# ETM-Code/eirgrid

Measured on AMD Instinct MI355X. Metric: 26-year episodes/sec, higher is better.
Workload: dtype f64

## Files before the change

eirgrid_amd/_native.py:

```python
from __future__ import annotations

import ctypes as C
import os

YEARS, N_ACTIONS, N_DEFICIT, N_COUNTS, N_TYPES = 26, 61, 15, 21, 15
GRID, CELLS, YEARLY_FIELDS = 51, 2601, 21
MAX_GENS, MAX_OFFSETS, RUN_CAP, DEF_CAP, ACT_CAP, ONCHIP_GENS = 4096, 4096, 4096, 4096, 4096, 512
TOPK_MAX = 64
PARETO_MAX = 256
PARETO_KEEP_SPREAD = 0x100
STATS_LEN = 8 + 2 * YEARS * N_ACTIONS + YEARS * N_DEFICIT
CANDIDATE_BYTES = 8 + 8 + 32 + 4 * YEARS + 4 * YEARS + RUN_CAP + DEF_CAP
PACKET_BYTES = 8 * STATS_LEN + CANDIDATE_BYTES

EG_OK, EG_ERR_NO_DEVICE, EG_ERR_BAD_ARG, EG_ERR_HIP, EG_ERR_UNSUPPORTED, EG_ERR_NOMEM, EG_ERR_INTERNAL = 0, -1, -2, -3, -4, -5, -6
EG_EP_OK, EG_EP_OVERFLOW, EG_EP_NO_LOCATION, EG_EP_INTERNAL = 0, -1, -2, -3

LIB_PATH = os.environ.get("EIRGRID_LIB") or os.path.join(os.path.dirname(os.path.abspath(__file__)), "libeirgrid_hip.so")

_dp = C.POINTER(C.c_double)
_u8p = C.POINTER(C.c_uint8)
_u16p = C.POINTER(C.c_uint16)
_u32p = C.POINTER(C.c_uint32)
_i32p = C.POINTER(C.c_int32)
# ... 123 lines not shown
DEBUG_TURNOVER_BREED, DEBUG_TURNOVER_EXPLORE = 1, 2
DEBUG_PARETO_ENTRY_BYTES = 56
DEBUG_PARETO_STATE_BYTES = 32 + PARETO_MAX * DEBUG_PARETO_ENTRY_BYTES
DEBUG_BREED_HEADER_BYTES, DEBUG_BREED_ROW_BYTES = 32, 288
DEBUG_BREED_READBACK_BYTES = DEBUG_BREED_HEADER_BYTES + PARETO_MAX * DEBUG_BREED_ROW_BYTES
DEBUG_BREED_BLOCK_OFFSETS = 416


class EgUpdateCandidate(C.Structure):
    _fields_ = [("score", C.c_double), ("index", C.c_int64), ("metrics", C.c_double * 4), ("n_run", C.c_int32 * YEARS), ("n_def", C.c_int32 * YEARS),
                ("run_log", C.c_uint8 * RUN_CAP), ("def_log", C.c_uint8 * DEF_CAP)]


class EgDebugRefineEntry(C.Structure):
    _fields_ = [("winner", C.c_int32), ("n_failed", C.c_int32), ("edit", C.c_uint32 * 2), ("score", C.c_double), ("metrics", C.c_double * 4),
                ("off26", C.c_int32), ("offd26", C.c_int32), ("base_ok", C.c_int32), ("n", C.c_int32), ("base_score", C.c_double),
                ("base_metrics", C.c_double * 4)]


assert C.sizeof(EgUpdateCandidate) == CANDIDATE_BYTES and C.sizeof(EgDebugRefineEntry) == 112

EXPORTS = [
    "eg_build_hash", "eg_last_error", "eg_device_count", "eg_create", "eg_destroy", "eg_rollout_batch", "eg_upload_snapshot",
    "eg_rollout_launch", "eg_rollout_launch_update", "eg_sync", "eg_last_batch_size", "eg_policy_hold", "eg_policy_rewind", "eg_replay_hoist", "eg_replay_hoist_stats", "eg_debug_hoist_stamps", "eg_fetch", "eg_timing_reset", "eg_timing_read", "eg_timing_read_grids", "eg_memory_report", "eg_update_stats", "eg_fetch_scores",
    "eg_fetch_episode_lists", "eg_fetch_record", "eg_fetch_best_run", "eg_best_result_track", "eg_fetch_best_result", "eg_evaluate_action_impact", "eg_place", "eg_find_suitable_location", "eg_debug_fill_lds", "eg_debug_occupy", "eg_policy_apply_reduced", "eg_policy_apply_packet", "eg_train_step",
    "eg_policy_push", "eg_device_rollout", "eg_device_apply", "eg_device_step", "eg_policy_pull",
    "eg_group_create", "eg_group_destroy", "eg_group_rank", "eg_group_push", "eg_group_step", "eg_group_pull", "eg_group_replay_hoist",
    "eg_group_best_result_track", "eg_group_fetch_best_result", "eg_top_k_track", "eg_fetch_top_k", "eg_rank_score",
    "eg_pareto_track", "eg_pareto_fold_last_batch", "eg_fetch_pareto", "eg_debug_pareto_fold",
    "eg_debug_load_batch", "eg_debug_fold_last_batch", "eg_debug_pick_best", "eg_debug_refine_pick",
    "eg_group_top_k_track", "eg_group_fetch_top_k", "eg_plans_validate", "eg_evaluate_plans", "eg_plans_load", "eg_plans_free",
    "eg_plan_edits_validate", "eg_evaluate_plan_edits", "eg_debug_fetch_plan_block", "eg_plans_save", "eg_refine_validate", "eg_refine_plan",
    "eg_refine_plans_validate", "eg_refine_plans", "eg_debug_refine_pick_many",
    "eg_debug_breed_begin", "eg_debug_breed_chunk", "eg_debug_breed_turnover", "eg_debug_breed_fetch",
    "eg_plan_moves_validate", "eg_evaluate_plan_moves", "eg_refine_plans_moves_validate", "eg_refine_plans_moves",
    "eg_plan_crosses_validate", "eg_evaluate_plan_crosses", "eg_plan_rewrites_validate", "eg_evaluate_plan_rewrites",
    "eg_breed_validate", "eg_breed_plans", "eg_explore_validate", "eg_explore_neighbourhood", "eg_explore_plans",
    "eg_host_tables_create", "eg_host_tables_free", "eg_host_tables_f64", "eg_host_tables_i32",
    "eg_policy_new", "eg_policy_free", "eg_policy_snapshot_view", "eg_policy_get_tables", "eg_policy_set_tables",
    "eg_policy_get_scalar", "eg_policy_set_scalar", "eg_policy_get_list", "eg_policy_apply_episode", "eg_score_metrics",
    "eg_policy_save_json", "eg_policy_load_json", "eg_policy_append_weight_history", "eg_policy_export_improvement_csv", "eg_export_summary_csv", "eg_export_run_details",
]

_lib = None


def source_hash() -> str:
    import glob
    import hashlib
    csrc = os.path.join(os.path.dirname(os.path.abspath(__file__)), "csrc")
    rel = [os.path.basename(f) for pat in ("*.hip", "*.cpp", "*.h") for f in glob.glob(os.path.join(csrc, pat))]
    rel += ["../../include/" + os.path.basename(f) for f in glob.glob(os.path.join(csrc, "..", "..", "include", "*.h"))]
    rel = sorted(set(rel + ["Makefile"]) - {"eg_build_hash.cpp"}, key=lambda r: r.encode())
    h = hashlib.sha256()
    for r in rel:
        h.update(open(os.path.join(csrc, r), "rb").read())
    return h.hexdigest()[:16]


def lib():
    global _lib
    if _lib is not None:
        return _lib
    if not os.path.exists(LIB_PATH):
        raise ImportError(f"{LIB_PATH} is missing: run `python -c 'import __graft_entry__ as g; g.build()'` "
                          "(hipcc --offload-arch=gfx950).  eirgrid_amd has no CPU fallback.")
    L = C.CDLL(LIB_PATH)
# ... 169 lines not shown
        L.eg_explore_neighbourhood.restype = C.c_int32
        L.eg_explore_neighbourhood.argtypes = [C.POINTER(EgPlanSet), C.POINTER(EgExploreOpts), C.POINTER(C.c_int64)]
        L.eg_explore_plans.restype = C.c_int32
        L.eg_explore_plans.argtypes = [C.c_void_p, C.POINTER(EgPolicySnapshot), C.POINTER(EgOpts), C.POINTER(EgPlanSet), C.POINTER(EgExploreOpts),
                                       C.c_uint64, C.c_uint64, C.POINTER(C.POINTER(EgPlanSet)), C.POINTER(EgExploreGeneration),
                                       C.POINTER(EgExploreMember), C.POINTER(C.c_int64), _i32p, _i32p, C.POINTER(EgEpisodeOut)]
    if hasattr(L, "eg_pareto_track") or not os.environ.get("EIRGRID_LIB"):
        L.eg_pareto_track.restype = C.c_int32
        L.eg_pareto_track.argtypes = [C.c_void_p, C.c_int32, C.c_int32, C.c_int32]
        L.eg_pareto_fold_last_batch.restype = C.c_int32
        L.eg_pareto_fold_last_batch.argtypes = [C.c_void_p]
        L.eg_fetch_pareto.restype = C.c_int32
        L.eg_fetch_pareto.argtypes = [C.c_void_p, C.POINTER(EgEpisodeOut), _i32p, C.POINTER(C.c_int64), _dp, C.POINTER(C.c_int64)]
        L.eg_debug_pareto_fold.restype = C.c_int32
        L.eg_debug_pareto_fold.argtypes = [C.c_void_p, _dp, _i32p, C.c_uint32, C.c_uint64]
    if hasattr(L, "eg_debug_load_batch") or not os.environ.get("EIRGRID_LIB"):
        L.eg_debug_load_batch.restype = C.c_int32
        L.eg_debug_load_batch.argtypes = [C.c_void_p, _dp, _i32p, _i32p, _u8p, _dp, C.c_uint32, C.c_uint64]
        L.eg_debug_fold_last_batch.restype = C.c_int32
        L.eg_debug_fold_last_batch.argtypes = [C.c_void_p, C.c_int32, C.c_int32]
        L.eg_debug_pick_best.restype = C.c_int32
        L.eg_debug_pick_best.argtypes = [C.c_void_p, C.c_void_p]
        L.eg_debug_refine_pick.restype = C.c_int32
        L.eg_debug_refine_pick.argtypes = [C.c_void_p, C.c_int32, C.c_void_p, _u8p]
    if hasattr(L, "eg_debug_breed_begin") or not os.environ.get("EIRGRID_LIB"):
        L.eg_debug_breed_begin.restype = C.c_int32
        L.eg_debug_breed_begin.argtypes = [C.c_void_p, C.c_int32, C.c_int32, C.c_int32]
        L.eg_debug_breed_chunk.restype = C.c_int32
        L.eg_debug_breed_chunk.argtypes = [C.c_void_p, _dp, _i32p, C.c_uint32, C.c_uint64]
        L.eg_debug_breed_turnover.restype = C.c_int32
        L.eg_debug_breed_turnover.argtypes = [C.c_void_p, C.c_int32, C.c_int32, C.c_int64]
        L.eg_debug_breed_fetch.restype = C.c_int32
        L.eg_debug_breed_fetch.argtypes = [C.c_void_p, C.c_void_p, _u8p, _u8p, _u8p, _u8p, C.c_void_p, _u64p]
    L.eg_plans_load.restype = C.POINTER(EgPlanSet)
    L.eg_plans_load.argtypes = [C.c_char_p]
    L.eg_plans_free.argtypes = [C.POINTER(EgPlanSet)]
    L.eg_rank_score.restype = C.c_double
    L.eg_rank_score.argtypes = [_dp, C.c_int32]
    L.eg_evaluate_action_impact.restype = C.c_double
    L.eg_evaluate_action_impact.argtypes = [_dp, _dp, C.c_int32]
    L.eg_fetch_best_run.restype = C.c_int32
    L.eg_fetch_best_run.argtypes = [C.c_void_p, C.POINTER(EgEpisodeOut), C.POINTER(C.c_int32)]
    L.eg_policy_export_improvement_csv.argtypes = [C.c_void_p, C.c_char_p]
    L.eg_find_suitable_location.restype = C.c_int32
    L.eg_find_suitable_location.argtypes = [C.c_void_p, C.c_int32, C.c_int32, _dp, _dp, C.c_int32, C.c_float, _dp, _dp, _i32p, _dp]
    L.eg_place.restype = C.c_int32
    L.eg_debug_fill_lds.restype = C.c_int32
    L.eg_debug_fill_lds.argtypes = [C.c_void_p, C.c_uint32]
    if hasattr(L, "eg_debug_occupy") or not os.environ.get("EIRGRID_LIB"):
        L.eg_debug_occupy.restype = C.c_int32
        L.eg_debug_occupy.argtypes = [C.c_void_p, C.c_int32, C.c_uint64]
    L.eg_place.argtypes = [C.c_void_p, C.c_int32, C.c_int32, _u16p, C.c_int32, _i32p, _dp]
    L.eg_host_tables_create.restype = C.c_void_p
    L.eg_host_tables_create.argtypes = [C.POINTER(EgWorld)]
    L.eg_host_tables_free.argtypes = [C.c_void_p]
    L.eg_host_tables_f64.restype = C.c_int32
    L.eg_host_tables_f64.argtypes = [C.c_void_p, C.c_char_p, C.POINTER(_dp), C.POINTER(C.c_int64)]
    L.eg_host_tables_i32.restype = C.c_int32
    L.eg_host_tables_i32.argtypes = [C.c_void_p, C.c_char_p, C.POINTER(_i32p), C.POINTER(C.c_int64)]
    L.eg_policy_new.restype = C.c_void_p
    L.eg_policy_free.argtypes = [C.c_void_p]
    L.eg_policy_snapshot_view.restype = C.c_int32
    L.eg_policy_snapshot_view.argtypes = [C.c_void_p, C.POINTER(EgPolicySnapshot)]
    L.eg_policy_get_tables.restype = C.c_int32
    L.eg_policy_get_tables.argtypes = [C.c_void_p, _dp, _dp, _dp]
    L.eg_policy_set_tables.restype = C.c_int32
# ... 28 lines not shown
```

eirgrid_amd/csrc/eg_api.cpp:

```cpp
#include <algorithm>
#include <cstdlib>
#include <cstring>

#include "eg_device_tables.h"
#include "eg_host.h"
#include "eg_policy_internal.h"

namespace eg {
namespace {
thread_local std::string g_error;
}
void set_error(const std::string& s) { g_error = s; }
}

using namespace eg;

void eg_host_tables::index() {
  auto F = [&](const char* n, const std::vector<double>& v) { f64[n] = {v.data(), (int64_t)v.size()}; };
  auto I = [&](const char* n, const std::vector<int32_t>& v) { i32[n] = {v.data(), (int64_t)v.size()}; };
  F("usage", H.usage); F("population", H.population); F("pre_co2", H.pre_co2); F("pre_tg", H.pre_tg); F("pre_ig", H.pre_ig);
  F("pre_sg", H.pre_sg); F("pre_optot", H.pre_optot); F("te", H.te); F("coastf", H.coastf); F("dr", H.dr); F("m03", H.m03);
  F("t12", H.t12); F("cc", H.cc); F("out_mw", H.out_mw); F("co2_t", H.co2_t); F("offv", H.offv); F("offc", H.offc);
  F("inflation", H.inflation); F("carbon_price", H.carbon_price);
  f64["size_factor"] = {&H.size_factor, 1};
  I("pre_opcnt", H.pre_opcnt); I("cls", H.cls); I("rclass", H.rclass); I("marine", H.marine); I("reach", H.reach);
  I("existing_online", H.existing_online);
}

namespace {
struct Options {
  bool helper_off = false, helper_all = false;
  bool heavy_slots_auto = true; uint32_t heavy_slots_wanted = 4096;
  uint32_t heavy_slots_max = 0;
  bool side_stream_plain = false;
  bool replay_hoist = false;
  int coop_force = 0;
  bool solo_on = true;
  uint32_t solo_tiles = 1u;
  uint32_t solo_lazy = 384u;
};
Options read_options() {
  Options o;
  if (const char* hv = std::getenv("EIRGRID_HELPER_WAVES")) { o.helper_off = std::string(hv) == "0"; o.helper_all = std::string(hv) == "all"; }
  if (const char* hs = std::getenv("EIRGRID_HEAVY_SLOTS")) { o.heavy_slots_wanted = (uint32_t)std::strtoul(hs, nullptr, 10); o.heavy_slots_auto = false; }
  o.heavy_slots_max = uint32_t((size_t(64) << 30) / (size_t(kRadiusClasses) * 2624 * sizeof(double)));
  if (const char* hg = std::getenv("EIRGRID_HEAVY_POOL_GB"))
    o.heavy_slots_max = uint32_t(std::min(double((1u << 20) - 1u), std::max(0.0, std::atof(hg)) * double(size_t(1) << 30) / double(size_t(kRadiusClasses) * 2624 * sizeof(double))));
  if (o.heavy_slots_max > (1u << 20) - 1u) o.heavy_slots_max = (1u << 20) - 1u;
  if (o.heavy_slots_wanted > o.heavy_slots_max) o.heavy_slots_wanted = o.heavy_slots_max;
  if (const char* sp = std::getenv("EIRGRID_SIDE_STREAM")) o.side_stream_plain = std::string(sp) == "plain";
  if (const char* rh = std::getenv("EIRGRID_REPLAY_HOIST")) o.replay_hoist = rh[0] == '1';
  if (const char* cf = std::getenv("EIRGRID_COOP_FORCE")) o.coop_force = std::atoi(cf);
  if (const char* so = std::getenv("EIRGRID_REPLAY_SOLO")) o.solo_on = so[0] != '0';
  if (const char* st = std::getenv("EIRGRID_SOLO_TILES")) o.solo_tiles = st[0] != '0' ? 1u : 0u;
  if (const char* sl = std::getenv("EIRGRID_SOLO_LAZY")) o.solo_lazy = std::string(sl) == "all" ? 0xFFFFFFFFu : (uint32_t)std::strtoul(sl, nullptr, 10);
  return o;
}

int collect_timing(eg_ctx* c, int count = -1) {
  if (count < 0 || count > c->ring_pending) count = c->ring_pending;
  for (; count > 0; --count) {
    const int i = (c->ring_head - c->ring_pending + 2 * eg_ctx::kTimingRing) % eg_ctx::kTimingRing;
    const bool heavy = c->ev_used[i] & 1, lean = c->ev_used[i] & 2;
    float best = 0.f, sum = 0.f;
    for (int a = 0; a < 2; ++a)
      for (int b = 0; b < 2; ++b) {
        if (!(a ? lean : heavy) || !(b ? lean : heavy)) continue;
        EG_HIP(hipEventSynchronize(c->ev[i][2 * b + 1]));
        float ms = 0.f;
        EG_HIP(hipEventElapsedTime(&ms, c->ev[i][2 * a], c->ev[i][2 * b + 1]));
        if (a == b) sum += ms;
        if (ms > best) best = ms;
// ... 521 lines not shown
```

eirgrid_amd/csrc/eg_debug.cpp:

```cpp
#include <cstring>

#include "eg_host.h"

using namespace eg;

namespace {
int refuse_rank(const eg_ctx* c, const char* who) {
  if (!c->group_member) return EG_OK;
  set_error(std::string(who) + ": the context is a rank of an eg_group (the test hooks have no group form)");
  return EG_ERR_BAD_ARG;
}
int put_field(eg_ctx* c, size_t field, const void* src, size_t width, uint32_t n) {
  EG_HIP(hipMemcpy2D(c->out.base + field, rec::stride, src, width, width, n, hipMemcpyHostToDevice));
  return EG_OK;
}
int refine_pick(eg_ctx* c, int32_t mode, const uint32_t* seg_first, const uint32_t* seg_count, int32_t n_segs, void* entries, uint8_t* base_blocks) {
  static_assert(sizeof(RefineEntry) == EG_DEBUG_REFINE_ENTRY_BYTES, "the step entry's layout is what the hooks document");
  static_assert(EG_PLAN_BLOCK_BYTES == snap::kPlanStride, "plan block");
  const uint32_t n = c->last_n;
  EG_HIP(hipSetDevice(c->device));
  constexpr size_t kWords = snap::kPlanStride / 4, kOff26 = (snap::best_off - snap::best_mask) / 4 + EG_YEARS, kOffD26 = (snap::bestd_off - snap::best_mask) / 4 + EG_YEARS;
  static_assert(kOff26 == 130 && kOffD26 == 158, "the words of the list totals as the hooks document them");
  const size_t S = size_t(n_segs);
  std::vector<uint32_t> blocks(size_t(n) * kWords), base(S * kWords), in(size_t(n) * 2 + S * 4);
// ... 86 lines not shown
  EG_TRY(ensure_packet(c));
  UpdateCandidate* d_cand = reinterpret_cast<UpdateCandidate*>(c->d_packet.ptr + 8 * EG_STATS_LEN);
  EG_HIP(hipMemsetAsync(d_cand, 0, sizeof(UpdateCandidate), nullptr));
  EG_LAUNCH("k_pick_best", launch_pick_best(c->out, c->last_n, c->last_first, d_cand, nullptr));
  EG_HIP(hipMemcpy(candidate, d_cand, sizeof(UpdateCandidate), hipMemcpyDeviceToHost));
  return EG_OK;
}

int32_t eg_debug_refine_pick(eg_ctx* c, int32_t mode, void* entry, uint8_t* base_block) {
  if (!c || !entry || !base_block || (mode != 1 && mode != 2)) { set_error("eg_debug_refine_pick: bad argument"); return EG_ERR_BAD_ARG; }
  EG_TRY(refuse_rank(c, "eg_debug_refine_pick"));
  const uint32_t first = 0, n = c->last_n;
  if (n == 0 || n > EG_REFINE_MAX_VARIANTS) { set_error("eg_debug_refine_pick: the last batch holds " + std::to_string(n) + " records (1..EG_REFINE_MAX_VARIANTS)"); return EG_ERR_BAD_ARG; }
  return refine_pick(c, mode, &first, &n, 1, entry, base_block);
}

int32_t eg_debug_refine_pick_many(eg_ctx* c, int32_t mode, const uint32_t* seg_first, const uint32_t* seg_count, int32_t n_segs, void* entries, uint8_t* base_blocks) {
  if (!c || !seg_first || !seg_count || !entries || !base_blocks || (mode != 1 && mode != 2)) { set_error("eg_debug_refine_pick_many: bad argument"); return EG_ERR_BAD_ARG; }
  EG_TRY(refuse_rank(c, "eg_debug_refine_pick_many"));
  const uint32_t n = c->last_n;
  if (n == 0 || n > EG_REFINE_MAX_VARIANTS) { set_error("eg_debug_refine_pick_many: the last batch holds " + std::to_string(n) + " records (1..EG_REFINE_MAX_VARIANTS)"); return EG_ERR_BAD_ARG; }
  if (n_segs < 1 || n_segs > EG_REFINE_MAX_PLANS) { set_error("eg_debug_refine_pick_many: n_segs = " + std::to_string(n_segs) + " (1..EG_REFINE_MAX_PLANS)"); return EG_ERR_BAD_ARG; }
  {
    uint64_t at = 0;
    for (int32_t s = 0; s < n_segs; ++s) {
      if (seg_first[s] != at || seg_count[s] == 0) { set_error("eg_debug_refine_pick_many: segment " + std::to_string(s) + " does not continue the tiling of the last batch"); return EG_ERR_BAD_ARG; }
      at += seg_count[s];
    }
    if (at != n) { set_error("eg_debug_refine_pick_many: the segments cover " + std::to_string(at) + " of the last batch's " + std::to_string(n) + " records"); return EG_ERR_BAD_ARG; }
  }
  return refine_pick(c, mode, seg_first, seg_count, n_segs, entries, base_blocks);
}

static_assert(sizeof(ParetoEntry) == EG_DEBUG_PARETO_ENTRY_BYTES && sizeof(ParetoState) == EG_DEBUG_PARETO_STATE_BYTES && offsetof(ParetoState, e) == 32,
              "the archive's state is what the hooks document");
static_assert(kBreedHeaderBytes == EG_DEBUG_BREED_HEADER_BYTES && kBreedRowBytes == EG_DEBUG_BREED_ROW_BYTES &&
              breed_at::kReadbackBytes == EG_DEBUG_BREED_READBACK_BYTES && snap::best_off - snap::best_mask == EG_DEBUG_BREED_BLOCK_OFFSETS &&
              sizeof(BreedCounters) == 16, "the readback buffer is what the hooks document");

int32_t eg_debug_breed_begin(eg_ctx* c, int32_t cap, int32_t objectives, int32_t mode) {
  if (!c) { set_error("eg_debug_breed_begin: bad argument"); return EG_ERR_BAD_ARG; }
  EG_TRY(refuse_rank(c, "eg_debug_breed_begin"));
  auto fail = [](const std::string& m) { set_error("eg_debug_breed_begin: " + m); return EG_ERR_BAD_ARG; };
  EG_TRY(check_cap(fail, cap)); EG_TRY(check_objectives(fail, objectives)); EG_TRY(check_mode(fail, mode));
  EG_HIP(hipSetDevice(c->device));
  c->debug_breed = false;
  static_assert(breed_at::records < breed_at::blocks && breed_at::blocks < breed_at::parents && breed_at::parents < breed_at::readback &&
                breed_at::readback + breed_at::kReadbackBytes == breed_at::counters, "the canary fills what lies between the state and the counters");
  EG_TRY(archive_begin(c, cap, objectives, mode, [c] {
    EG_HIP(hipMemset(c->d_breed + breed_at::records, EG_DEBUG_BREED_CANARY, breed_at::counters - breed_at::records));
    return EG_OK;
  }));
  c->debug_breed = true;
  return EG_OK;
}

int32_t eg_debug_breed_chunk(eg_ctx* c, const double* metrics, const int32_t* status, uint32_t n, uint64_t first_index) {
  if (!c || !metrics || !status) { set_error("eg_debug_breed_chunk: bad argument"); return EG_ERR_BAD_ARG; }
  EG_TRY(refuse_rank(c, "eg_debug_breed_chunk"));
  if (!c->debug_breed) { set_error("eg_debug_breed_chunk: eg_debug_breed_begin first"); return EG_ERR_BAD_ARG; }
  if (n == 0 || n > EG_CROSS_MAX_VARIANTS) { set_error("eg_debug_breed_chunk: n = " + std::to_string(n) + " (1..EG_CROSS_MAX_VARIANTS)"); return EG_ERR_BAD_ARG; }
  if (first_index > uint64_t(INT64_MAX) - n) { set_error("eg_debug_breed_chunk: first_index + n passes 2^63 (an entry's index is an int64)"); return EG_ERR_BAD_ARG; }
  EG_TRY(eg_debug_load_batch(c, metrics, status, nullptr, nullptr, nullptr, n, first_index));
  constexpr size_t kWords = snap::kPlanStride / 4;
  std::vector<uint32_t> blocks(size_t(n) * kWords);
  for (uint32_t j = 0; j < n; ++j) {
// ... 40 lines not shown
```

eirgrid_amd/csrc/eg_field.h:

```cpp
#pragma once

constexpr int kHeavyGens = 8;
constexpr int kFieldStride = 2624;
constexpr int kSearchFallback = -3;
typedef unsigned int u32x4 __attribute__((ext_vector_type(4)));
typedef const u32x4 __attribute__((address_space(1)))* GlobalVec4;
typedef double __attribute__((address_space(1)))* GlobalF64;
typedef const double __attribute__((address_space(1)))* GlobalF64c;
__device__ __forceinline__ PsRec load_rec(unsigned long long list_addr, int i) {
  const GlobalVec4 p = (GlobalVec4)(list_addr + (unsigned long long)(unsigned)i * sizeof(PsRec));
  const u32x4 lo = p[0], hi = p[1];
  PsRec r;
  __builtin_memcpy(&r, &lo, 16); __builtin_memcpy(reinterpret_cast<char*>(&r) + 16, &hi, 16);
  return r;
}
typedef const int __attribute__((address_space(1)))* GlobalI32c;
__device__ __forceinline__ double field_load(GlobalF64 p) {
  return __hip_atomic_load(p, __ATOMIC_RELAXED, __HIP_MEMORY_SCOPE_AGENT);
}
template <bool kLatency>
__device__ __forceinline__ double factor_by_q(int rc, int table, int q) {
  if constexpr (kLatency) return sl.dr16[2 * (rc * kD2Stride + q)];
  else return *reinterpret_cast<const double*>(reinterpret_cast<const char*>(&sm) + ((table & 0xFFFF) + q * 8));
}
// ... 223 lines not shown
    if ((m1 >> lane) & 1ull) sm.gstage[1][__popcll(m1 & ((1ull << lane) - 1ull))] = (__double2loint(lm) & 63) * kWave + lane;
  } else {
    for (int k = 0; k < K; ++k) {
      const double approx = pb_at(k * kWave + lane) * field_at(pc_at(k * kWave + lane));
      const unsigned long long m = __ballot(approx >= thr && approx > 0.0);
      if (m != 0ull) {
        const int pos = ncand + __popcll(m & ((1ull << lane) - 1ull));
        if (((m >> lane) & 1ull) && pos < kWave) sm.gstage[1][pos] = k * kWave + lane;
        ncand += __popcll(m);
      }
    }
  }
  if (ncand > kWave || ncand == 0) return kSearchFallback;
  wave_sync();
#ifdef EG_STAMPS
  asm volatile("s_waitcnt vmcnt(0)" ::: "memory");
  const unsigned long long ts2 = __builtin_readcyclecounter();
#endif
  const ChunkBest b = heavy_exact<kLatency>(list_addr, tail_cells, size_factor, lane, rc, tbl, ngen_s, ncand, ncand == 1 && solo >= 0 ? __builtin_amdgcn_readlane(lcell, solo) : -1);
  if (!(b.score > 0.0)) return kSearchFallback;
#ifdef EG_STAMPS
  if (lane == 0) { sm.hdbg[0][0] += ts1 - ts0; sm.hdbg[0][1] += ts2 - ts1; sm.hdbg[0][2] += __builtin_readcyclecounter() - ts2; sm.hdbg[1][0] += (unsigned long long)K; sm.hdbg[1][1] += (unsigned long long)ncand; sm.hdbg[1][2] += 1ull; }
#endif
  return heavy_result(b, lane, K, ncand);
}

constexpr int kTilesUndecided = -4;
static_assert(kTileW * kTileW == kWave, "a cell of a tile per lane");
constexpr int kNoTile = 63;
static_assert(kNoTile >= kTiles && (kNoTile / kTileCols) * kTileW >= kGrid, "kNoTile is off the grid");

constexpr int kTileCounters = kCells + 1;
static_assert((kFieldStride - kTileCounters) * 8 >= kTiles * 2 && EG_MAX_GENS <= 0xFFFF, "a 16-bit counter per tile fits behind a class's cells");
__device__ __forceinline__ int tiles_refresh(unsigned long long a_s, int applied, int ta, int tb, int lane, int rc, int tbl, int reach, int ngen_s,
                                             unsigned long long tail_cells, double& fa, double& fb) {
  const int cap = factor_cap<false>(tbl);
  const int ra = (ta / kTileCols) * kTileW, ca = (ta % kTileCols) * kTileW, rb = (tb / kTileCols) * kTileW, cb = (tb % kTileCols) * kTileW;
  const int ia = ra + (lane >> 3), ja = ca + (lane & 7), ib = rb + (lane >> 3), jb = cb + (lane & 7);
  const int aa = __builtin_amdgcn_readlane(applied, ta), ab = tb < kTiles ? __builtin_amdgcn_readlane(applied, tb) : ngen_s;
  fa = aa == 0 ? 1.0 : fa; fb = ab == 0 ? 1.0 : fb;
  int folded = 0;
  const unsigned span = (unsigned)(kTileW - 1 + 2 * reach);
  for (int gb = (aa < ab ? aa : ab) & ~(kWave - 1); gb < ngen_s; gb += kWave) {
    const int gc = list_cell(tail_cells, gb, lane, ngen_s, 0), g = gb + lane;
    const int gi = gc / kGrid, gj = gc - gi * kGrid;
    const bool na = g >= aa && g < ngen_s && (unsigned)(gi - ra + reach) <= span && (unsigned)(gj - ca + reach) <= span;
    const bool nb = g >= ab && g < ngen_s && (unsigned)(gi - rb + reach) <= span && (unsigned)(gj - cb + reach) <= span;
    const int gij = gi | (gj << 8);
    unsigned long long near = __ballot(na || nb);
    while (near != 0ull) {
      const int j = __ffsll((long long)near) - 1;
      const int w = __builtin_amdgcn_readlane(gij, j), si = w & 255, sj = w >> 8;
      int qa = (ia - si) * (ia - si) + (ja - sj) * (ja - sj), qb = (ib - si) * (ib - si) + (jb - sj) * (jb - sj);
      qa = qa < cap && gb + j >= aa ? qa : cap;
      qb = qb < cap && gb + j >= ab ? qb : cap;
      fa = fa * factor_by_q<false>(rc, tbl, qa);
      fb = fb * factor_by_q<false>(rc, tbl, qb);
      near &= near - 1ull;
      ++folded;
    }
  }
  if (ia < kGrid && ja < kGrid) *(GlobalF64)(a_s + (unsigned long long)((unsigned)(ia * kGrid + ja) * 8u)) = fa;
  if (ib < kGrid && jb < kGrid) *(GlobalF64)(a_s + (unsigned long long)((unsigned)(ib * kGrid + jb) * 8u)) = fb;
  if (lane == 0) {
    const GlobalU16 cnt = (GlobalU16)(a_s + 8ull * kTileCounters);
    cnt[ta] = (unsigned short)ngen_s;
    if (tb < kTiles) cnt[tb] = (unsigned short)ngen_s;
  }
  return folded;
}
__device__ __noinline__ void tiles_catch_up_all(unsigned long long class_addr, unsigned long long tail_cells, int lane, int rc, int tbl, int reach, int ngen) {
  asm volatile("s_waitcnt vmcnt(0)" ::: "memory");
  const int ngen_s = __builtin_amdgcn_readfirstlane(ngen);
  const unsigned long long a_s = ((unsigned long long)(unsigned)__builtin_amdgcn_readfirstlane((int)(class_addr >> 32)) << 32) | (unsigned)__builtin_amdgcn_readfirstlane((int)class_addr);
  const int applied = lane < kTiles ? tail_u16(a_s + 8ull * kTileCounters, lane) : 0;
  if (__ballot(lane < kTiles && applied != ngen_s) == 0ull) return;
#pragma nounroll
  for (int ta = 0; ta < kTiles; ta += 2) {
    const int tb = ta + 1 < kTiles ? ta + 1 : kNoTile;
    const int ia = (ta / kTileCols) * kTileW + (lane >> 3), ja = (ta % kTileCols) * kTileW + (lane & 7);
    const int ib = (tb / kTileCols) * kTileW + (lane >> 3), jb = (tb % kTileCols) * kTileW + (lane & 7);
    const int ca = ia < kGrid && ja < kGrid ? ia * kGrid + ja : 0, cb = ib < kGrid && jb < kGrid ? ib * kGrid + jb : 0;
    double fa = field_load((GlobalF64)a_s + ca), fb = field_load((GlobalF64)a_s + cb);
    tiles_refresh(a_s, applied, ta, tb, lane, rc, tbl, reach, ngen_s, tail_cells, fa, fb);
  }
}

template <bool kLazy>
__device__ __noinline__ int place_tiles(unsigned long long tab_addr, int yv, unsigned long long class_addr, unsigned long long tiles_addr,
                                        unsigned long long tail_cells, double size_factor, int lane, int rc_in, int tbl, int ngen) {
  const int rc = kLazy ? rc_in & 255 : rc_in, reach = kLazy ? rc_in >> 8 : 0;
#ifdef EG_STAMPS
  const unsigned long long ts0 = __builtin_readcyclecounter();
// ... 157 lines not shown
```

eirgrid_amd/csrc/eg_internal.h:

```cpp
#pragma once
#include <cstddef>
#include <cstdint>
#include <string>
#include <vector>

#include "eirgrid_hip.h"

namespace eg {

constexpr int kYears = EG_YEARS;
constexpr int kTypes = EG_N_TYPES;
constexpr int kCells = EG_CELLS;
constexpr int kGrid = EG_GRID;
constexpr int kRadiusClasses = 6;
constexpr int kMaxReach = 12;
constexpr int kMults = 3;
constexpr int kOffsetTypes = 4;
constexpr int kPsStride = 2624;
constexpr int kDrCompact = 352;
constexpr int kLdsGens = EG_ONCHIP_GENS;
constexpr int kShortReplayMax = 96;
constexpr int kMaxVariants = 12;
constexpr int kTileW = 8;
constexpr int kTileCols = (kGrid + kTileW - 1) / kTileW;
// ... 223 lines not shown
  const uint32_t* d_index;
  uint32_t off, period;
  void* ev[4];
  unsigned long long hoist_seq;
  HoistInfo* d_hoist;
  uint8_t* coop_out;
  int coop_force;
  long long* d_stats_rep;
  unsigned long long solo_seq;
  unsigned long long* d_solo;
  bool plans;
  uint32_t n_short;
  const uint32_t* d_index_long;
  bool same_index;
};
constexpr int kStatsReplicas = 64;
int launch_fold_stats(long long* d_rep, long long* d_stats, void* stream);
struct HoistInfo {
  unsigned long long served_seq;
  unsigned long long coop_seq;
  int32_t lens[6];
  int32_t pad[2];
  int32_t g_end[EG_YEARS], o_end[EG_YEARS];
  unsigned long long bytes;
  int32_t books_done, pad2;
  double year[EG_YEARS][8];
  unsigned long long stamps[8];
};
constexpr size_t kHoistBytes = (sizeof(HoistInfo) + 63) & ~size_t(63);
int launch_rollout(const DevTables& t, const DevSnapshot& s, const DevOut& o, uint64_t seed, uint64_t first_index,
                   uint32_t n, const uint8_t* d_replay_mask, uint32_t replay_period, long long* d_stats, const RolloutPlan& plan);
int launch_fill_lds(uint32_t value, uint32_t* d_sink, int n_workgroups, void* stream);
int launch_occupy(int variant, unsigned long long cycles, uint32_t* d_sink, void* stream);
int launch_stalled_tables(uint8_t* d_snap, void* stream);
int launch_rewind(uint8_t* d_snap, const uint8_t* d_held, uint32_t* list_len_out, void* stream);
int launch_apply_update(uint8_t* d_snap, const void* d_packets, int n_packets, size_t packet_stride, long long* d_zero_stats, uint64_t noise_seed,
                        const DevOut& o, uint32_t n_local, uint64_t first_index, bool local_pick, uint32_t* list_len_out, void* stream);
int launch_place(const DevTables& t, int gen_type, int year_index, const uint16_t* d_cells, int n_extra,
                 int32_t* d_out_cell, double* d_out_score, void* stream);
int launch_place_xy(const DevTables& t, int gen_type, int year_index, const double* d_x, const double* d_y, int n, double radius,
                    double size_term, int32_t* d_out_cell, double* d_out_score, void* stream);
double class_radius(int radius_class);
struct StatsParams {
  double best_score;
  int32_t has_best;
  double threshold;
  int32_t forced;
  double adaptive_lr;
  double stagnation;
};
int launch_update_stats(const DevSnapshot& s, const DevOut& o, uint32_t n, long long* d_stats, void* stream);
struct UpdateCandidate {
  double score;
  long long index;
  double metrics[4];
  int32_t n_run[EG_YEARS], n_def[EG_YEARS];
  uint8_t run_log[EG_RUN_CAP], def_log[EG_DEF_CAP];
};
static_assert(sizeof(UpdateCandidate) == EG_CANDIDATE_BYTES, "candidate layout is part of the C ABI");
int launch_pick_best(const DevOut& o, uint32_t n, uint64_t first_index, UpdateCandidate* d_cand, void* stream);
struct FoldState { double metrics[4]; long long index; int32_t has, pad; };
constexpr size_t kFoldRecord = 64;
constexpr size_t kFoldBytes = kFoldRecord + rec::stride;
static_assert(sizeof(FoldState) <= kFoldRecord, "fold state layout");
int launch_fold_best(const DevOut& o, uint32_t n, uint64_t first_index, bool cost_only, uint8_t* d_fold, void* stream);
struct FoldEntry { double net, opinion, cost; int32_t ok, pad; };
// ... 114 lines not shown
```

eirgrid_amd/csrc/eg_replay_solo.h:

```cpp
#pragma once

namespace solo {

struct Lists {
  unsigned long long gen_pack;
  __device__ __forceinline__ static int* words() { return reinterpret_cast<int*>(sm.pol); }
  __device__ __forceinline__ int gpack_at(int i) const {
    __builtin_amdgcn_fence(__ATOMIC_RELEASE, "workgroup");
    return tail_u16(gen_pack, i);
  }
  __device__ __forceinline__ void gpack_put(int, int) const {}
  __device__ __forceinline__ void opack_put(int, int) const {}
  __device__ __forceinline__ int cls(int t) const { return (sm.type_info[t] >> 12) & 3; }
  __device__ __forceinline__ double out(int t) const { return sm.type_out[t]; }
  __device__ __forceinline__ void year_end(int yi, int ngen, int noff) const { words()[yi] = ngen; words()[EG_YEARS + yi] = noff; }
  __device__ __forceinline__ void finish(int run_pos, int def_pos, int act_pos, int ngen, int noff, unsigned long long bytes) const {
    int* w = words();
    w[52] = run_pos; w[53] = def_pos; w[54] = act_pos; w[55] = ngen; w[56] = noff;
    *reinterpret_cast<unsigned long long*>(w + 58) = bytes;
  }
};
static_assert(snap::kPolRow * 8 >= 60 * 4, "the script's lengths fit the policy row block");

constexpr int kEnt = 8;
// ... 191 lines not shown
  if (stats != nullptr) {
    __builtin_amdgcn_fence(__ATOMIC_RELEASE, "workgroup");
    __builtin_amdgcn_fence(__ATOMIC_ACQUIRE, "workgroup");
    wave_sync();
    StatsParams P;
    load_stats_params(S, P);
    episode_update_stats(O, S, P, e, lane, stats, 1ull, emap.stats_rep ? (int)(blockIdx.x % (uint32_t)kStatsReplicas) : -1);
  }
  EG_SS(6);
#ifdef EG_SOLO_STAMPS
  if (lane == 0) {
    unsigned long long* dbg = (unsigned long long*)(O.act_log(e) + EG_ACT_CAP - 256);
    for (int i = 0; i < 8; ++i) dbg[i] = cs[i];
#ifdef EG_STAMPS
    for (int i = 0; i < 3; ++i) { dbg[8 + i] = sm.hdbg[0][i]; dbg[11 + i] = sm.hdbg[1][i]; }
    dbg[14] = sm.hdbg[1][3];
    dbg[15] = sm.hdbg[0][3];
#endif
  }
#endif
  if (lane == 0) emap.solo[blockIdx.x] = emap.solo_seq;
}

__global__ void __launch_bounds__(kWave, EG_HEAVY_WAVES) k_replay_solo(DevTables T, DevSnapshot S_in, DevOut O, unsigned long long first_index, uint32_t n_episodes,
                                                                       const uint8_t* __restrict__ replay_mask, uint32_t replay_period, long long* stats,
                                                                       EpisodeMap emap) {
  replay_solo_episode<false>(T, S_in, O, first_index, n_episodes, replay_mask, replay_period, stats, emap);
}
__global__ void __launch_bounds__(kWave, EG_HEAVY_WAVES) k_replay_lazy(DevTables T, DevSnapshot S_in, DevOut O, unsigned long long first_index, uint32_t n_episodes,
                                                                       const uint8_t* __restrict__ replay_mask, uint32_t replay_period, long long* stats,
                                                                       EpisodeMap emap) {
  replay_solo_episode<true>(T, S_in, O, first_index, n_episodes, replay_mask, replay_period, stats, emap);
}
```

eirgrid_amd/csrc/eg_rollout.hip:

```cpp
#include <hip/hip_runtime.h>
#include <cstddef>
#include <hip/hip_ext.h>

#include "eg_internal.h"

#define EG_DETPOW_QUAL __device__ __forceinline__
#include "eg_detpow.h"
#define EG_RM __device__ __forceinline__
#include "eg_reduced_math.h"

namespace eg {
namespace {

constexpr int kWave = 64;
constexpr int kD2Max = 144, kD2Stride = 146;
constexpr int kCmdYear = 1 << 30;
constexpr int kHelperWaves = 1;
constexpr int kSpinCap = 1 << 20;
constexpr int kSearchLost = -2;
constexpr double kMinWeight = 0.0001;
constexpr double kMaxWeight = 0.999;
constexpr double kMaxCost = 50000000000.0;
constexpr int kBattery = 12, kPeaker = 8;
constexpr int kNothing = 60, kFirstOffset = 45, kFirstOther = 57;
// ... 1584 lines not shown

#include "eg_update_kernels.h"
#endif
}

int launch_rollout_throughput(int kind, const DevTables& t, const DevSnapshot& s, const DevOut& o, uint64_t seed, uint64_t first_index, uint32_t n,
                              const uint8_t* d_replay_mask, uint32_t replay_period, long long* d_stats, uint32_t count, uint32_t mode,
                              const uint32_t* index, uint32_t off, uint32_t period, const unsigned long long* hoist, unsigned long long hoist_seq,
                              uint32_t stats_rep, uint32_t same_index, unsigned long long* solo, unsigned long long solo_seq, void* stream, void* ev0, void* ev1);
#ifdef EG_TU_THROUGHPUT
int launch_rollout_throughput(int kind, const DevTables& t, const DevSnapshot& s, const DevOut& o, uint64_t seed, uint64_t first_index, uint32_t n,
                              const uint8_t* d_replay_mask, uint32_t replay_period, long long* d_stats, uint32_t count, uint32_t mode,
                              const uint32_t* index, uint32_t off, uint32_t period, const unsigned long long* hoist, unsigned long long hoist_seq,
                              uint32_t stats_rep, uint32_t same_index, unsigned long long* solo, unsigned long long solo_seq, void* stream, void* ev0, void* ev1) {
  EpisodeMap map{};
  map.count = count; map.mode = mode; map.index = index; map.off = off; map.period = period; map.hoist = hoist; map.hoist_seq = hoist_seq; map.stats_rep = stats_rep; map.same_index = same_index;
  map.solo = solo; map.solo_seq = solo_seq;
#define EG_LAUNCH_TP(kKind) hipExtLaunchKernelGGL((k_rollout<0, kKind>), dim3(map.count), dim3(kWave), 0, (hipStream_t)stream, (hipEvent_t)ev0, (hipEvent_t)ev1, 0, \
                                                  t, s, o, (unsigned long long)seed, (unsigned long long)first_index, n, d_replay_mask, replay_period, d_stats, map)
  if (kind == kReplayLong) {
    if (solo_seq != 0ull && t.solo_tiles != 0u && t.solo_lazy != 0u)
      hipLaunchKernelGGL(k_replay_lazy, dim3(map.count), dim3(kWave), 0, (hipStream_t)stream, t, s, o, (unsigned long long)first_index, n, d_replay_mask, replay_period,
                         d_stats, map);
    else if (solo_seq != 0ull)
      hipLaunchKernelGGL(k_replay_solo, dim3(map.count), dim3(kWave), 0, (hipStream_t)stream, t, s, o, (unsigned long long)first_index, n, d_replay_mask, replay_period,
                         d_stats, map);
    EG_LAUNCH_TP(kReplayLong);
  }
  else if (kind == kReplayShort) EG_LAUNCH_TP(kReplayShort);
  else EG_LAUNCH_TP(kLean);
#undef EG_LAUNCH_TP
  return (int)hipGetLastError();
}
#else
namespace {
template <int kKind>
void launch_variant(bool helper_waves, const DevTables& t, const DevSnapshot& s, const DevOut& o, uint64_t seed, uint64_t first_index, uint32_t n,
                    const uint8_t* d_replay_mask, uint32_t replay_period, long long* d_stats, const EpisodeMap& map, void* stream, void* ev0, void* ev1) {
  if (helper_waves)
    hipExtLaunchKernelGGL((k_rollout<kHelperWaves, kKind>), dim3(map.count), dim3(kWave * (1 + kHelperWaves)), 0, (hipStream_t)stream,
                          (hipEvent_t)ev0, (hipEvent_t)ev1, 0, t, s, o, (unsigned long long)seed, (unsigned long long)first_index, n,
                          d_replay_mask, replay_period, d_stats, map);
  else
    (void)launch_rollout_throughput(kKind, t, s, o, seed, first_index, n, d_replay_mask, replay_period, d_stats, map.count, map.mode, map.index, map.off, map.period,
                                    map.hoist, map.hoist_seq, map.stats_rep, map.same_index, map.solo, map.solo_seq, stream, ev0, ev1);
}
}

int launch_rollout(const DevTables& t, const DevSnapshot& s, const DevOut& o, uint64_t seed, uint64_t first_index,
                   uint32_t n, const uint8_t* d_replay_mask, uint32_t replay_period, long long* d_stats_packet, const RolloutPlan& p) {
  if (n == 0) return 0;
  const bool rep = d_stats_packet != nullptr && p.d_stats_rep != nullptr;
  long long* d_stats = rep ? p.d_stats_rep : d_stats_packet;
  if (p.plans) {
    EpisodeMap ms{}, ml{};
    ms.count = p.n_short; ms.mode = 1u; ms.index = p.d_index;
    ml.count = p.n_heavy - p.n_short; ml.mode = 1u; ml.index = p.d_index_long;
    ms.same_index = ml.same_index = p.same_index ? 1u : 0u;
    if (!p.helper_waves && p.solo_seq != 0ull) { ml.solo = p.d_solo; ml.solo_seq = p.solo_seq; }
    if (ms.count > 0) launch_variant<kReplayShort>(p.helper_waves, t, s, o, seed, first_index, n, d_replay_mask, replay_period, d_stats, ms, p.stream_heavy, p.ev[0],
                                                   ml.count > 0 ? nullptr : p.ev[1]);
    else (void)hipEventRecord((hipEvent_t)p.ev[0], (hipStream_t)p.stream_heavy);
    if (ml.count > 0) launch_variant<kReplayLong>(p.helper_waves, t, s, o, seed, first_index, n, d_replay_mask, replay_period, d_stats, ml, p.stream_heavy, nullptr, p.ev[1]);
    return (int)hipGetLastError();
  }
  if (p.n_heavy > 0) {
// ... 261 lines not shown
```

include/eirgrid_hip.h:

```cpp
#ifndef EIRGRID_HIP_H
#define EIRGRID_HIP_H

#include <stdint.h>

#ifdef __cplusplus
extern "C" {
#endif

#define EG_YEARS 26
#define EG_N_ACTIONS 61
#define EG_N_DEFICIT 15
#define EG_N_COUNTS 21
#define EG_N_TYPES 15
#define EG_GRID 51
#define EG_CELLS (EG_GRID * EG_GRID)
#define EG_YEARLY_FIELDS 21

#define EG_MAX_GENS 4096
#define EG_MAX_OFFSETS 4096
#define EG_RUN_CAP 4096
#define EG_DEF_CAP 4096
#define EG_ACT_CAP 4096
#define EG_ONCHIP_GENS 512

// ... 254 lines not shown
int32_t eg_group_fetch_best_result(eg_group *, eg_episode_out *out, int32_t *state, int64_t *global_index);
int32_t eg_group_top_k_track(eg_group *, int32_t k, int32_t mode);
int32_t eg_group_fetch_top_k(eg_group *, eg_episode_out *out, int32_t *n_held, double *scores, int64_t *global_index);

int32_t eg_debug_fill_lds(eg_ctx *, uint32_t value);
#define EG_DEBUG_LIST_LEN 8
#define EG_DEBUG_FOLD_BEST_RESULT 1
#define EG_DEBUG_FOLD_TOP_K 2
#define EG_DEBUG_REFINE_ENTRY_BYTES 112
int32_t eg_debug_load_batch(eg_ctx *, const double *metrics , const int32_t *status , const int32_t *n_act ,
                            const uint8_t *act_log , const double *score_list , uint32_t n,
                            uint64_t first_index);
int32_t eg_debug_fold_last_batch(eg_ctx *, int32_t what, int32_t use_score_list);
int32_t eg_debug_pick_best(eg_ctx *, void *candidate );
int32_t eg_debug_refine_pick(eg_ctx *, int32_t mode , void *entry , uint8_t *base_block );
int32_t eg_debug_refine_pick_many(eg_ctx *, int32_t mode, const uint32_t *seg_first, const uint32_t *seg_count, int32_t n_segs,
                                  void *entries , uint8_t *base_blocks );
#define EG_DEBUG_BREED_CANARY 0xC5
#define EG_DEBUG_BREED_TAG_MUL 0x9E3779B97F4A7C15ull
#define EG_DEBUG_TURNOVER_BREED 1
#define EG_DEBUG_TURNOVER_EXPLORE 2
#define EG_DEBUG_PARETO_ENTRY_BYTES 56
#define EG_DEBUG_PARETO_STATE_BYTES (32 + EG_PARETO_MAX * EG_DEBUG_PARETO_ENTRY_BYTES)
#define EG_DEBUG_BREED_HEADER_BYTES 32
#define EG_DEBUG_BREED_ROW_BYTES 288
#define EG_DEBUG_BREED_READBACK_BYTES (EG_DEBUG_BREED_HEADER_BYTES + EG_PARETO_MAX * EG_DEBUG_BREED_ROW_BYTES)
#define EG_DEBUG_BREED_BLOCK_OFFSETS 416
int32_t eg_debug_breed_begin(eg_ctx *, int32_t cap, int32_t objectives, int32_t mode);
int32_t eg_debug_breed_chunk(eg_ctx *, const double *metrics , const int32_t *status , uint32_t n, uint64_t first_index);
int32_t eg_debug_breed_turnover(eg_ctx *, int32_t kind, int32_t next, int64_t m_first);
int32_t eg_debug_breed_fetch(eg_ctx *, void *state , uint8_t *blocks ,
                             uint8_t *array0 , uint8_t *array1 ,
                             uint8_t *readback , void *counters , uint64_t *tags );
int32_t eg_debug_occupy(eg_ctx *, int32_t variant, uint64_t cycles);

int32_t eg_place(eg_ctx *, int32_t gen_type, int32_t year_index, const uint16_t *extra_cells, int32_t n_extra ,
                 int32_t *out_cell, double *out_score);

int32_t eg_find_suitable_location(eg_ctx *, int32_t year_index, int32_t gen_type, const double *gen_x, const double *gen_y,
                                  int32_t n_generators, float size_penalty, double *out_x, double *out_y, int32_t *found,
                                  double *out_score );

typedef struct eg_host_tables eg_host_tables;
eg_host_tables *eg_host_tables_create(const eg_world *world);
void eg_host_tables_free(eg_host_tables *);
int32_t eg_host_tables_f64(const eg_host_tables *, const char *name, const double **ptr, int64_t *len);
int32_t eg_host_tables_i32(const eg_host_tables *, const char *name, const int32_t **ptr, int64_t *len);

eg_policy *eg_policy_new(void);
void eg_policy_free(eg_policy *);
int32_t eg_policy_snapshot_view(const eg_policy *, eg_policy_snapshot *out);
int32_t eg_policy_get_tables(const eg_policy *, double *w, double *dw, double *cw);
int32_t eg_policy_set_tables(eg_policy *, const double *w, const double *dw, const double *cw);
double eg_policy_get_scalar(const eg_policy *, int32_t which);
int32_t eg_policy_set_scalar(eg_policy *, int32_t which, double v);
int32_t eg_policy_get_list(const eg_policy *, int32_t which, int32_t year_index, uint8_t *out, int32_t cap);
int32_t eg_policy_apply_episode(eg_policy *, const double metrics[4], const int32_t *n_run, const uint8_t *run_log,
                                const int32_t *n_def, const uint8_t *def_log, uint64_t noise_seed);
int32_t eg_policy_apply_reduced(eg_policy *, const int64_t *stats, const double cand_metrics[4], const int32_t *cand_n_run,
                                const uint8_t *cand_run_log, const int32_t *cand_n_def, const uint8_t *cand_def_log,
                                uint64_t noise_seed);
int32_t eg_policy_apply_packet(eg_policy *, const int64_t *stats, const void *candidates, int32_t n_candidates,
                               uint64_t noise_seed);
int32_t eg_train_step(eg_ctx *, eg_policy *, const eg_opts *opts, uint64_t seed, uint64_t first_episode_index,
                      uint32_t n_episodes, const uint8_t *replay_mask , uint64_t noise_seed);
int32_t eg_policy_push(eg_ctx *, const eg_policy *, const eg_opts *opts);
// ... 25 lines not shown
```

Measured before the change: 9.583 million.

## Compact near generators into LDS rows and fold tile factors in pairs

```diff
diff --git a/eirgrid_amd/_native.py b/eirgrid_amd/_native.py
--- a/eirgrid_amd/_native.py
+++ b/eirgrid_amd/_native.py
@@ -179,7 +179,7 @@
     "eg_group_top_k_track", "eg_group_fetch_top_k", "eg_plans_validate", "eg_evaluate_plans", "eg_plans_load", "eg_plans_free",
     "eg_plan_edits_validate", "eg_evaluate_plan_edits", "eg_debug_fetch_plan_block", "eg_plans_save", "eg_refine_validate", "eg_refine_plan",
     "eg_refine_plans_validate", "eg_refine_plans", "eg_debug_refine_pick_many",
-    "eg_debug_breed_begin", "eg_debug_breed_chunk", "eg_debug_breed_turnover", "eg_debug_breed_fetch",
+    "eg_debug_breed_begin", "eg_debug_breed_chunk", "eg_debug_breed_turnover", "eg_debug_breed_fetch", "eg_debug_tiles_refresh",
     "eg_plan_moves_validate", "eg_evaluate_plan_moves", "eg_refine_plans_moves_validate", "eg_refine_plans_moves",
     "eg_plan_crosses_validate", "eg_evaluate_plan_crosses", "eg_plan_rewrites_validate", "eg_evaluate_plan_rewrites",
     "eg_breed_validate", "eg_breed_plans", "eg_explore_validate", "eg_explore_neighbourhood", "eg_explore_plans",
@@ -415,6 +415,9 @@
         L.eg_debug_breed_turnover.argtypes = [C.c_void_p, C.c_int32, C.c_int32, C.c_int64]
         L.eg_debug_breed_fetch.restype = C.c_int32
         L.eg_debug_breed_fetch.argtypes = [C.c_void_p, C.c_void_p, _u8p, _u8p, _u8p, _u8p, C.c_void_p, _u64p]
+    if hasattr(L, "eg_debug_tiles_refresh") or not os.environ.get("EIRGRID_LIB"):
+        L.eg_debug_tiles_refresh.restype = C.c_int32
+        L.eg_debug_tiles_refresh.argtypes = [C.c_void_p, _u16p, C.c_int32, C.c_int32, C.c_int32, C.c_int32, _dp, _i32p]
     L.eg_plans_load.restype = C.POINTER(EgPlanSet)
     L.eg_plans_load.argtypes = [C.c_char_p]
     L.eg_plans_free.argtypes = [C.POINTER(EgPlanSet)]
diff --git a/eirgrid_amd/csrc/eg_api.cpp b/eirgrid_amd/csrc/eg_api.cpp
--- a/eirgrid_amd/csrc/eg_api.cpp
+++ b/eirgrid_amd/csrc/eg_api.cpp
@@ -37,7 +37,7 @@
   int coop_force = 0;
   bool solo_on = true;
   uint32_t solo_tiles = 1u;
-  uint32_t solo_lazy = 384u;
+  uint32_t solo_lazy = 512u;
 };
 Options read_options() {
   Options o;
diff --git a/eirgrid_amd/csrc/eg_debug.cpp b/eirgrid_amd/csrc/eg_debug.cpp
--- a/eirgrid_amd/csrc/eg_debug.cpp
+++ b/eirgrid_amd/csrc/eg_debug.cpp
@@ -142,6 +142,30 @@
   return refine_pick(c, mode, seg_first, seg_count, n_segs, entries, base_blocks);
 }
 
+int32_t eg_debug_tiles_refresh(eg_ctx* c, const uint16_t* cells, int32_t n_cells, int32_t radius_class, int32_t tile_a, int32_t tile_b, double* field, int32_t* folded) {
+  if (!c || !field || !folded || (n_cells > 0 && !cells)) { set_error("eg_debug_tiles_refresh: bad argument"); return EG_ERR_BAD_ARG; }
+  EG_TRY(refuse_rank(c, "eg_debug_tiles_refresh"));
+  auto fail = [](const std::string& m) { set_error("eg_debug_tiles_refresh: " + m); return EG_ERR_BAD_ARG; };
+  if (n_cells < 0 || n_cells > EG_MAX_GENS) return fail("n_cells = " + std::to_string(n_cells) + " (0..EG_MAX_GENS)");
+  for (int32_t i = 0; i < n_cells; ++i) if (cells[i] >= kCells) return fail("cells[" + std::to_string(i) + "] = " + std::to_string(cells[i]) + " is not a grid cell");
+  if (tile_a < 0 || tile_a >= kTiles || tile_b < -1 || tile_b >= kTiles || tile_b == tile_a) return fail("tiles " + std::to_string(tile_a) + ", " + std::to_string(tile_b) + " (0..48, distinct; tile_b -1: none)");
+  bool has_class = false;
+  for (int t = 0; t < kTypes; ++t) has_class = has_class || c->tables.H.rclass[t] == radius_class;
+  if (radius_class < 0 || radius_class >= kRadiusClasses || !has_class) return fail("radius_class " + std::to_string(radius_class) + " is no generator type's");
+  EG_HIP(hipSetDevice(c->device));
+  DevBuf<double> d_field; DevBuf<uint16_t> d_cells; DevBuf<int> d_out;
+  EG_HIP(d_field.reserve(EG_DEBUG_FIELD_DOUBLES)); EG_HIP(d_cells.reserve(size_t(EG_MAX_GENS))); EG_HIP(d_out.reserve(1));
+  EG_HIP(hipMemcpy(d_field, field, sizeof(double) * EG_DEBUG_FIELD_DOUBLES, hipMemcpyHostToDevice));
+  if (n_cells > 0) EG_HIP(hipMemcpy(d_cells, cells, sizeof(uint16_t) * size_t(n_cells), hipMemcpyHostToDevice));
+  EG_LAUNCH("k_debug_tiles_refresh", launch_debug_tiles_refresh(c->dev, d_field, d_cells, n_cells, radius_class, tile_a, tile_b, d_out, nullptr));
+  int out = 0;
+  EG_HIP(hipMemcpy(&out, d_out, sizeof(int), hipMemcpyDeviceToHost));
+  EG_HIP(hipMemcpy(field, d_field, sizeof(double) * EG_DEBUG_FIELD_DOUBLES, hipMemcpyDeviceToHost));
+  if (out < 0) return fail("the device found no generator type of radius class " + std::to_string(radius_class));
+  *folded = out;
+  return EG_OK;
+}
+
 static_assert(sizeof(ParetoEntry) == EG_DEBUG_PARETO_ENTRY_BYTES && sizeof(ParetoState) == EG_DEBUG_PARETO_STATE_BYTES && offsetof(ParetoState, e) == 32,
               "the archive's state is what the hooks document");
 static_assert(kBreedHeaderBytes == EG_DEBUG_BREED_HEADER_BYTES && kBreedRowBytes == EG_DEBUG_BREED_ROW_BYTES &&
diff --git a/eirgrid_amd/csrc/eg_field.h b/eirgrid_amd/csrc/eg_field.h
--- a/eirgrid_amd/csrc/eg_field.h
+++ b/eirgrid_amd/csrc/eg_field.h
@@ -279,33 +279,62 @@
 
 constexpr int kTileCounters = kCells + 1;
 static_assert((kFieldStride - kTileCounters) * 8 >= kTiles * 2 && EG_MAX_GENS <= 0xFFFF, "a 16-bit counter per tile fits behind a class's cells");
+static_assert(sizeof(sm.gstage[0]) >= (kWave + 2) * sizeof(int) && sizeof(sm.gstage[0]) % 8 == 0, "a row's padding and read-ahead stay inside the row");
+constexpr int kGenPadFar = (int)0xC000C000;
 __device__ __forceinline__ int tiles_refresh(unsigned long long a_s, int applied, int ta, int tb, int lane, int rc, int tbl, int reach, int ngen_s,
                                              unsigned long long tail_cells, double& fa, double& fb) {
-  const int cap = factor_cap<false>(tbl);
+  (void)rc;
+  const int dr_off = tbl & 0xFFFF, cap = factor_cap<false>(tbl);
   const int ra = (ta / kTileCols) * kTileW, ca = (ta % kTileCols) * kTileW, rb = (tb / kTileCols) * kTileW, cb = (tb % kTileCols) * kTileW;
   const int ia = ra + (lane >> 3), ja = ca + (lane & 7), ib = rb + (lane >> 3), jb = cb + (lane & 7);
+  const short2v cpa = __builtin_bit_cast(short2v, ia | (ja << 16)), cpb = __builtin_bit_cast(short2v, ib | (jb << 16));
   const int aa = __builtin_amdgcn_readlane(applied, ta), ab = tb < kTiles ? __builtin_amdgcn_readlane(applied, tb) : ngen_s;
   fa = aa == 0 ? 1.0 : fa; fb = ab == 0 ? 1.0 : fb;
   int folded = 0;
   const unsigned span = (unsigned)(kTileW - 1 + 2 * reach);
+  const int2* rowa = reinterpret_cast<const int2*>(sm.gstage[0]);
+  const int2* rowb = reinterpret_cast<const int2*>(sm.gstage[1]);
   for (int gb = (aa < ab ? aa : ab) & ~(kWave - 1); gb < ngen_s; gb += kWave) {
     const int gc = list_cell(tail_cells, gb, lane, ngen_s, 0), g = gb + lane;
     const int gi = gc / kGrid, gj = gc - gi * kGrid;
     const bool na = g >= aa && g < ngen_s && (unsigned)(gi - ra + reach) <= span && (unsigned)(gj - ca + reach) <= span;
     const bool nb = g >= ab && g < ngen_s && (unsigned)(gi - rb + reach) <= span && (unsigned)(gj - cb + reach) <= span;
-    const int gij = gi | (gj << 8);
-    unsigned long long near = __ballot(na || nb);
-    while (near != 0ull) {
-      const int j = __ffsll((long long)near) - 1;
-      const int w = __builtin_amdgcn_readlane(gij, j), si = w & 255, sj = w >> 8;
-      int qa = (ia - si) * (ia - si) + (ja - sj) * (ja - sj), qb = (ib - si) * (ib - si) + (jb - sj) * (jb - sj);
-      qa = qa < cap && gb + j >= aa ? qa : cap;
-      qb = qb < cap && gb + j >= ab ? qb : cap;
-      fa = fa * factor_by_q<false>(rc, tbl, qa);
-      fb = fb * factor_by_q<false>(rc, tbl, qb);
-      near &= near - 1ull;
-      ++folded;
-    }
+    const unsigned long long ma = __ballot(na), mb = __ballot(nb);
+    if ((ma | mb) == 0ull) continue;
+    const int gp = gi | (gj << 16);
+    if (na) sm.gstage[0][__builtin_amdgcn_mbcnt_hi((unsigned)(ma >> 32), __builtin_amdgcn_mbcnt_lo((unsigned)ma, 0u))] = gp;
+    if (nb) sm.gstage[1][__builtin_amdgcn_mbcnt_hi((unsigned)(mb >> 32), __builtin_amdgcn_mbcnt_lo((unsigned)mb, 0u))] = gp;
+    const int cnt_a = __popcll(ma), cnt_b = __popcll(mb);
+    if (lane == 0) { sm.gstage[0][cnt_a] = kGenPadFar; sm.gstage[1][cnt_b] = kGenPadFar; }
+    asm volatile("" ::: "memory");
+    folded += __popcll(ma | mb);
+    const int pairs_a = (cnt_a + 1) >> 1, pairs_b = (cnt_b + 1) >> 1, both = pairs_a < pairs_b ? pairs_a : pairs_b;
+    if (both > 0) {
+      double a0, a1, b0, b1;
+      int2 ga = rowa[0], gq = rowb[0];
+#pragma nounroll
+      for (int k = 0; k < both; ++k) {
+        a0 = factor_at(cpa, ga.x, dr_off, cap); b0 = factor_at(cpb, gq.x, dr_off, cap); a1 = factor_at(cpa, ga.y, dr_off, cap); b1 = factor_at(cpb, gq.y, dr_off, cap);
+        __builtin_amdgcn_sched_barrier(0);
+        ga = rowa[k + 1]; gq = rowb[k + 1];
+        fa = fa * a0; fb = fb * b0; fa = fa * a1; fb = fb * b1;
+      }
+    }
+#define EG_TR_REST(row2, cpk, s, n_pairs)                                                                                          \
+    {                                                                                                                              \
+      double a0, a1;                                                                                                               \
+      int2 gcur = row2[both];                                                                                                      \
+      _Pragma("nounroll") for (int k = both; k < n_pairs; ++k) {                                                                   \
+        a0 = factor_at(cpk, gcur.x, dr_off, cap); a1 = factor_at(cpk, gcur.y, dr_off, cap);                                        \
+        __builtin_amdgcn_sched_barrier(0);                                                                                         \
+        gcur = row2[k + 1];                                                                                                        \
+        s = s * a0; s = s * a1;                                                                                                    \
+      }                                                                                                                            \
+    }
+    if (pairs_a > both) EG_TR_REST(rowa, cpa, fa, pairs_a)
+    else if (pairs_b > both) EG_TR_REST(rowb, cpb, fb, pairs_b)
+#undef EG_TR_REST
+    asm volatile("" ::: "memory");
   }
   if (ia < kGrid && ja < kGrid) *(GlobalF64)(a_s + (unsigned long long)((unsigned)(ia * kGrid + ja) * 8u)) = fa;
   if (ib < kGrid && jb < kGrid) *(GlobalF64)(a_s + (unsigned long long)((unsigned)(ib * kGrid + jb) * 8u)) = fb;
diff --git a/eirgrid_amd/csrc/eg_internal.h b/eirgrid_amd/csrc/eg_internal.h
--- a/eirgrid_amd/csrc/eg_internal.h
+++ b/eirgrid_amd/csrc/eg_internal.h
@@ -279,6 +279,7 @@
                    uint32_t n, const uint8_t* d_replay_mask, uint32_t replay_period, long long* d_stats, const RolloutPlan& plan);
 int launch_fill_lds(uint32_t value, uint32_t* d_sink, int n_workgroups, void* stream);
 int launch_occupy(int variant, unsigned long long cycles, uint32_t* d_sink, void* stream);
+int launch_debug_tiles_refresh(const DevTables& t, double* d_field, const uint16_t* d_cells, int n_cells, int radius_class, int tile_a, int tile_b, int* d_out, void* stream);
 int launch_stalled_tables(uint8_t* d_snap, void* stream);
 int launch_rewind(uint8_t* d_snap, const uint8_t* d_held, uint32_t* list_len_out, void* stream);
 int launch_apply_update(uint8_t* d_snap, const void* d_packets, int n_packets, size_t packet_stride, long long* d_zero_stats, uint64_t noise_seed,
diff --git a/eirgrid_amd/csrc/eg_replay_solo.h b/eirgrid_amd/csrc/eg_replay_solo.h
--- a/eirgrid_amd/csrc/eg_replay_solo.h
+++ b/eirgrid_amd/csrc/eg_replay_solo.h
@@ -247,3 +247,21 @@
                                                                        EpisodeMap emap) {
   replay_solo_episode<true>(T, S_in, O, first_index, n_episodes, replay_mask, replay_period, stats, emap);
 }
+__global__ void __launch_bounds__(kWave, EG_HEAVY_WAVES) k_debug_tiles_refresh(DevTables T, unsigned long long field_addr, unsigned long long cells_addr, int n_cells, int rc,
+                                                                               int ta, int tb, int* out) {
+  const int lane = threadIdx.x;
+  load_static_tables(T, lane, true);
+  for (int i = lane; i < kLdsGens && i < n_cells; i += kWave) sm.gcell[i] = (uint16_t)tail_u16(cells_addr, i);
+  wave_sync();
+  int info = 0, type = -1;
+  for (int t = kTypes - 1; t >= 0; --t) { const int w = sm.type_info[t]; if (((w >> 4) & 15) == rc) { info = w; type = t; } }
+  info = __builtin_amdgcn_readfirstlane(info);
+  if (__builtin_amdgcn_readfirstlane(type) < 0) { if (lane == 0) out[0] = -1; return; }
+  const int applied = lane < kTiles ? tail_u16(field_addr + 8ull * kTileCounters, lane) : 0;
+  const int ia = (ta / kTileCols) * kTileW + (lane >> 3), ja = (ta % kTileCols) * kTileW + (lane & 7);
+  const int ib = (tb / kTileCols) * kTileW + (lane >> 3), jb = (tb % kTileCols) * kTileW + (lane & 7);
+  const int ca = ia < kGrid && ja < kGrid ? ia * kGrid + ja : 0, cb = ib < kGrid && jb < kGrid ? ib * kGrid + jb : 0;
+  double fa = field_load((GlobalF64)field_addr + ca), fb = field_load((GlobalF64)field_addr + cb);
+  const int folded = tiles_refresh(field_addr, applied, ta, tb, lane, rc, throughput_table(info), (info >> 8) & 15, __builtin_amdgcn_readfirstlane(n_cells), cells_addr, fa, fb);
+  if (lane == 0) out[0] = folded;
+}
diff --git a/eirgrid_amd/csrc/eg_rollout.hip b/eirgrid_amd/csrc/eg_rollout.hip
--- a/eirgrid_amd/csrc/eg_rollout.hip
+++ b/eirgrid_amd/csrc/eg_rollout.hip
@@ -1640,6 +1640,13 @@
 #undef EG_LAUNCH_TP
   return (int)hipGetLastError();
 }
+int launch_debug_tiles_refresh(const DevTables& t, double* d_field, const uint16_t* d_cells, int n_cells, int radius_class, int tile_a, int tile_b, int* d_out, void* stream) {
+  static_assert(kFieldStride == EG_DEBUG_FIELD_DOUBLES && kTileCounters == EG_DEBUG_TILE_COUNTERS && kTiles == EG_DEBUG_TILES && kTileW == EG_DEBUG_TILE_WIDTH,
+                "the class field is what the hook documents");
+  hipLaunchKernelGGL(k_debug_tiles_refresh, dim3(1), dim3(kWave), 0, (hipStream_t)stream, t, (unsigned long long)d_field, (unsigned long long)d_cells, n_cells, radius_class,
+                     tile_a, tile_b < 0 ? kNoTile : tile_b, d_out);
+  return (int)hipGetLastError();
+}
 #else
 namespace {
 template <int kKind>
diff --git a/include/eirgrid_hip.h b/include/eirgrid_hip.h
--- a/include/eirgrid_hip.h
+++ b/include/eirgrid_hip.h
@@ -310,6 +310,12 @@
 int32_t eg_debug_breed_fetch(eg_ctx *, void *state , uint8_t *blocks ,
                              uint8_t *array0 , uint8_t *array1 ,
                              uint8_t *readback , void *counters , uint64_t *tags );
+#define EG_DEBUG_FIELD_DOUBLES 2624
+#define EG_DEBUG_TILE_COUNTERS 2602
+#define EG_DEBUG_TILES 49
+#define EG_DEBUG_TILE_WIDTH 8
+int32_t eg_debug_tiles_refresh(eg_ctx *, const uint16_t *cells , int32_t n_cells, int32_t radius_class, int32_t tile_a, int32_t tile_b,
+                               double *field , int32_t *folded);
 int32_t eg_debug_occupy(eg_ctx *, int32_t variant, uint64_t cycles);
 
 int32_t eg_place(eg_ctx *, int32_t gen_type, int32_t year_index, const uint16_t *extra_cells, int32_t n_extra ,
```

Result: faster. 9.792 million (median of 6 runs) (+2.2%).
